# tmuird/VAEUNET

Hardware: AMD Instinct MI355X
Metric: images/sec (whole node) at 3x512x512 bs=8/GPU; Dice parity vs CPU ref (higher is better)
Workload: dtype bf16; 1 GPU; UNet(3,2) train step (fwd+CombinedLoss+bwd+clip+AdamW), random-init weights; image=3x512x512, batch_per_gpu=8, global_batch=8, parallelism=dp1, execution=hipgraph-replay, wgrad_side_stream=False

## Files before the change

include/vaeunet.h:

```cpp
#ifndef VAEUNET_H
#define VAEUNET_H
#include <stdint.h>
#ifdef __cplusplus
extern "C" {
#endif

typedef struct VuGather {
  const void* src[3];
  int64_t stride[3];
  int32_t cend[3];
  int32_t nsrc;
  int32_t C;
  int32_t N, H, W;
  int32_t Hs, Ws;
  int32_t R, S;
  int32_t sy, sx, dy, dx, oy, ox;
} VuGather;

typedef struct VuGemmFwd {
  VuGather a;
  const void* b;
  int64_t ldb;
  int32_t ncol;
  int32_t out_mode;
// ... 170 lines not shown
                     const float* coef2, void* dx1, int64_t dx1s, void* dx2, int64_t dx2s, int dtype,
                     void* stream);
int vu_conv_image_wgrad_bn_ok(int C, int Cp, int64_t das, int64_t ys, int64_t imgs, int N, int H, int W,
                              int dtype);
int vu_conv_image_wgrad_bn_slabs(int N, int H, int W);
int vu_conv_image_wgrad_bn(const void* da, int64_t das, const void* y, int64_t ys, const float* scale,
                           const float* shift, const float* mean, const float* k, int relu,
                           const void* img, int64_t imgs, int N, int H, int W, float* slab, int nslab,
                           void* stream);

int vu_chan_sum(const void* x, int64_t stride, int N, int H, int W, int y0,
                int x0, int Hr, int Wr, int C, float* out, int accumulate,
                float* workspace, int dtype, void* stream);
int64_t vu_reduce_workspace_bytes(int64_t P, int C);
int64_t vu_bn_finalize_workspace_bytes(int tiles, int C);
int vu_zero(void* y, int64_t ys, int64_t P, int C, int dtype, void* stream);
int vu_gpu_delay(int rounds, void* stream);
int vu_zero_insert2(const void* dy, int64_t dys, int N, int h, int w, int C,
                    void* up, int64_t ups, int H, int W, int dtype, void* stream);
int vu_copy(const void* x, int64_t xs, int xdtype, void* y, int64_t ys,
            int ydtype, int64_t P, int C, int accumulate, void* stream);
int vu_input_pack(const float* x, int64_t sn, int64_t sc, int64_t sh,
                  int64_t sw, int N, int C, int H, int W, int Cp, void* y,
                  int dtype, void* stream);

int vu_maxpool2_fwd(const void* x, int64_t xs, int N, int H, int W, int C,
                    void* y, int64_t ys, int dtype, void* stream);
int vu_maxpool2_bwd(const void* x, int64_t xs, const void* dy, int64_t dys,
                    int N, int H, int W, int C, void* dx, int64_t dxs,
                    const void* add, int64_t adds, int dtype, void* stream);
int vu_bn_apply_maxpool2(const void* y, int64_t ys, void* a, int64_t as, void* pool, int64_t ps,
                         int N, int H, int W, int C, const float* scale, const float* shift,
                         int relu, int dtype, void* stream);
int vu_upsample_fwd(const void* x, int64_t xs, int N, int Hi, int Wi, int C,
                    void* y, int64_t ys, int Ho, int Wo, int Hp, int Wp,
                    int py, int px, int dtype, void* stream);
int vu_upsample_bwd(const void* dy, int64_t dys, int N, int Hi, int Wi, int C,
                    void* dx, int64_t dxs, int Ho, int Wo, int Hp, int Wp,
                    int py, int px, int accumulate, int dtype, void* stream);

int64_t vu_attn_tile_rows(void);
int vu_attn_psi_fwd(const void* ug, const void* ux, int64_t P, int F,
                    const float* sg, const float* tg, const float* sx,
                    const float* tx, const float* wpsi, const float* bpsi,
                    float* q, float* psum, float* pm2, int64_t tile_rows,
                    int dtype, void* stream);
int vu_attn_gate_fwd(const float* q, const float* st, const void* x,
                     int64_t xs, int64_t P, int C, float* pmap, void* out,
                     int64_t os, int dtype, void* stream);
int vu_attn_gate_bwd(const void* dout, int64_t dos, const void* x, int64_t xs,
                     const float* pmap, int64_t P, int C, void* dx,
                     int64_t dxs, float* dqpre, int dtype, void* stream);
int64_t vu_attn_psi_bwd_workspace_bytes(int64_t P, int F);
int vu_attn_psi_bwd(const void* ug, const void* ux, int64_t P, int F,
                    const float* sg, const float* tg, const float* sx,
                    const float* tx, const float* wpsi, const float* dq,
                    void* ds, float* dwpsi, float* dbpsi, int accumulate,
                    float* workspace, int dtype, void* stream);
int64_t vu_attn_psi_bwd_blocks(int64_t P);
int vu_attn_psi_bwd_bnb_ok(int F);
int vu_attn_psi_bwd_bnb(const void* ug, const void* ux, int64_t P, int F,
                        const float* sg, const float* tg, const float* sx,
                        const float* tx, const float* wpsi, const float* dq,
                        void* ds, float* dwpsi, float* dbpsi, int accumulate,
                        float* workspace, const float* mean_g, const float* invstd_g,
                        const float* mean_x, const float* invstd_x, float* bnb_g,
// ... 271 lines not shown
```

vaeunet_amd/_lib.py:

```python
import ctypes as C
import os

import torch

_HERE = os.path.dirname(os.path.abspath(__file__))
LIB_PATH = os.path.join(_HERE, "libvaeunet_hip.so")
if os.environ.get("VU_LIB_PATH"):
    LIB_PATH = os.environ["VU_LIB_PATH"]

F32, BF16 = 0, 1

_p = C.c_void_p
_i = C.c_int
_l = C.c_int64
_f = C.c_float


class VuGather(C.Structure):
    _fields_ = [("src", _p * 3), ("stride", _l * 3), ("cend", C.c_int32 * 3),
                ("nsrc", C.c_int32), ("C", C.c_int32),
                ("N", C.c_int32), ("H", C.c_int32), ("W", C.c_int32),
                ("Hs", C.c_int32), ("Ws", C.c_int32), ("R", C.c_int32), ("S", C.c_int32),
                ("sy", C.c_int32), ("sx", C.c_int32), ("dy", C.c_int32), ("dx", C.c_int32),
                ("oy", C.c_int32), ("ox", C.c_int32)]
# ... 84 lines not shown
    "vu_permute4_tile": (_l, []),
    "vu_permute4_batch": (_i, [_p, _i, _l, _p]),
    "vu_permute4_batch2": (_i, [_p, _i, _i, _l, _l, _p]),
    "vu_permute4": (_i, [_p, _l, _l, _l, _l, _l, _i, _i, _i, _i, _i, _p, _i, _p]),
    "vu_bn_finalize": (_i, [_p, _p, _i, _l, _l, _i, _p, _p, _p, _p, _f, _f, _p, _p, _p, _p,
                            _p, _p, _p]),
    "vu_bn_finalize_workspace_bytes": (_l, [_i, _i]),
    "vu_bn_eval_coeffs": (_i, [_p, _p, _p, _p, _f, _i, _p, _p, _p, _p, _p]),
    "vu_bn_apply": (_i, [_p, _l, _p, _l, _l, _i, _p, _p, _i, _i, _p]),
    "vu_bn_fwd_fused_supported": (_i, [_i, _i, _l, _l, _l]),
    "vu_bn_bwd_fused_supported": (_i, [_l, _i, _l, _l, _l]),
    "vu_bn_bwd_fused": (_i, [_p, _l, _p, _l, _l, _i, _p, _p, _p, _p, _p, _i, _i, _p, _p, _i, _p, _l, _p, _i,
                             _p]),
    "vu_bn_fwd_fused": (_i, [_p, _p, _i, _l, _l, _i, _p, _p, _p, _p, _p, _f, _f, _p, _p, _l, _p, _l, _p, _p,
                             _p, _l, _i, _i, _p]),
    "vu_bn_bwd_reduce": (_i, [_p, _l, _p, _l, _l, _i, _p, _p, _p, _p, _p, _i, _i, _p, _p, _i,
                              _p, _p, _i, _p]),
    "vu_bn_bwd_apply": (_i, [_p, _l, _p, _l, _l, _i, _p, _p, _p, _p, _i, _p, _l, _i, _p]),
    "vu_bn_bwd_apply2_ok": (_i, [_i, _l, _l, _l, _l, _l]),
    "vu_bn_bwd_apply2": (_i, [_p, _l, _p, _l, _p, _l, _l, _i, _p, _p, _p, _p, _p, _l, _p, _l, _i, _p]),
    "vu_conv_image_wgrad_bn_ok": (_i, [_i, _i, _l, _l, _l, _i, _i, _i, _i]),
    "vu_conv_image_wgrad_bn_slabs": (_i, [_i, _i, _i]),
    "vu_conv_image_wgrad_bn": (_i, [_p, _l, _p, _l, _p, _p, _p, _p, _i, _p, _l, _i, _i, _i, _p, _i, _p]),
    "vu_reduce_workspace_bytes": (_l, [_l, _i]),
    "vu_chan_sum": (_i, [_p, _l, _i, _i, _i, _i, _i, _i, _i, _i, _p, _i, _p, _i, _p]),
    "vu_copy": (_i, [_p, _l, _i, _p, _l, _i, _l, _i, _i, _p]),
    "vu_zero": (_i, [_p, _l, _l, _i, _i, _p]),
    "vu_gpu_delay": (_i, [_i, _p]),
    "vu_zero_insert2": (_i, [_p, _l, _i, _i, _i, _i, _p, _l, _i, _i, _i, _p]),
    "vu_input_pack": (_i, [_p, _l, _l, _l, _l, _i, _i, _i, _i, _i, _p, _i, _p]),
    "vu_maxpool2_fwd": (_i, [_p, _l, _i, _i, _i, _i, _p, _l, _i, _p]),
    "vu_maxpool2_bwd": (_i, [_p, _l, _p, _l, _i, _i, _i, _i, _p, _l, _p, _l, _i, _p]),
    "vu_bn_apply_maxpool2": (_i, [_p, _l, _p, _l, _p, _l, _i, _i, _i, _i, _p, _p, _i, _i, _p]),
    "vu_upsample_fwd": (_i, [_p, _l, _i, _i, _i, _i, _p, _l, _i, _i, _i, _i, _i, _i, _i, _p]),
    "vu_upsample_bwd": (_i, [_p, _l, _i, _i, _i, _i, _p, _l, _i, _i, _i, _i, _i, _i, _i, _i,
                             _p]),
    "vu_attn_tile_rows": (_l, []),
    "vu_attn_psi_fwd": (_i, [_p, _p, _l, _i, _p, _p, _p, _p, _p, _p, _p, _p, _p, _l, _i, _p]),
    "vu_attn_gate_fwd": (_i, [_p, _p, _p, _l, _l, _i, _p, _p, _l, _i, _p]),
    "vu_attn_gate_bwd": (_i, [_p, _l, _p, _l, _p, _l, _i, _p, _l, _p, _i, _p]),
    "vu_attn_psi_bwd_workspace_bytes": (_l, [_l, _i]),
    "vu_attn_psi_bwd_blocks": (_l, [_l]),
    "vu_attn_psi_bwd_bnb_ok": (_i, [_i]),
    "vu_attn_psi_bwd_bnb": (_i, [_p, _p, _l, _i, _p, _p, _p, _p, _p, _p, _p, _p, _p, _i, _p, _p, _p, _p, _p, _p, _p,
                                 _i, _p]),
    "vu_attn_psi_bwd": (_i, [_p, _p, _l, _i, _p, _p, _p, _p, _p, _p, _p, _p, _p, _i, _p, _i,
                             _p]),
    "vu_attn_tail_bwd_tile": (_l, [_i, _i]),
    "vu_attn_tail_bwd_ok": (_i, [_l, _i, _i, _l, _l, _l, _l, _l, _l, _i]),
    "vu_attn_tail_bwd": (_i, [_p, _p, _p, _l, _i, _i, _p, _p, _p, _p, _p, _p, _p, _p, _p, _p, _l, _p, _l, _p, _l,
                              _p, _p, _l, _l, _i, _p, _l, _p, _p, _i, _p]),
    "vu_pointwise_fwd": (_i, [_p, _l, _l, _i, _i, _p, _p, _p, _l, _i, _p]),
    "vu_pointwise_bwd_workspace_bytes": (_l, [_l, _i, _i]),
    "vu_pointwise_bn_fwd": (_i, [_p, _l, _l, _i, _i, _p, _p, _p, _p, _p, _l, _i, _p]),
    "vu_pointwise_bn_bwd_blocks": (_l, [_l]),
    "vu_pointwise_bn_bwd": (_i, [_p, _l, _p, _l, _p, _l, _l, _i, _i, _p, _p, _l, _p, _p, _i, _p, _p, _i, _p]),
    "vu_pointwise_bwd": (_i, [_p, _l, _p, _l, _l, _i, _i, _p, _p, _l, _p, _p, _i, _p, _i, _p]),
    "vu_loss_workspace_bytes": (_l, []),
    "vu_bce_dice_fwd2": (_i, [_p, _p, _l, _p, _f, _f, _f, _p, _p, _p, _p]),
    "vu_bce_dice_bwd": (_i, [_p, _p, _l, _p, _f, _f, _f, _p, _p, _p]),
    "vu_focal_workspace_bytes": (_l, []),
    "vu_focal_dice_fwd": (_i, [_p, _p, _l, _f, _f, _f, _f, _f, _i, _p, _p, _p, _p, _p]),
    "vu_focal_dice_bwd": (_i, [_p, _p, _l, _f, _f, _f, _f, _f, _i, _p, _p, _p, _p]),
    "vu_kl_free_bits2": (_i, [_p, _p, _i, _i, _f, _p, _p, _p, _p, _p]),
    "vu_sumsq": (_i, [_p, _l, _p, _p, _p]),
    "vu_dice_score": (_i, [_p, _p, _l, _f, _p, _p, _p, _p]),
# ... 95 lines not shown
```

vaeunet_amd/csrc/bn.hip:

```cpp
#include <cstdlib>
#include <type_traits>

#include "host.h"
#include "bn_bwd_elem.h"

namespace {

constexpr int STATS_TPB = 32;
constexpr int STATS_MAXS = 256;

__global__ void bn_stats_stage1(const float* psum, const float* pm2, int tiles, int64_t tile_rows,
                                int64_t rows, int C, int S, double* ws) {
  __shared__ double sh[4][64];
  const int cl = threadIdx.x & 63, tl = threadIdx.x >> 6;
  const int c = blockIdx.x * 64 + cl;
  const bool ok = c < C;
  const int per = (tiles + S - 1) / S;
  const int tb0 = blockIdx.y * per, te0 = min(tiles, tb0 + per);
  constexpr int U = STATS_TPB / 4;
  double N = 0, Mn = 0, Q = 0;
  for (int tb = tb0; tb < te0; tb += STATS_TPB) {
    const int te = min(te0, tb + STATS_TPB);
    const int64_t n_r = min(rows, (int64_t)te * tile_rows) - (int64_t)tb * tile_rows;
    float sv[U], mv[U];
// ... 403 lines not shown
      o2.store(dx2 + p * dx2s + c);
    }
  }
}

template <typename T>
__global__ void bn_bwd_apply_scalar(const T* dy, int64_t dys, const T* x, int64_t xs, int64_t P, int C,
                                    const float* scale, const float* shift, const float* mean,
                                    const float* coef, int relu, T* dx, int64_t dxs) {
  int64_t tot = P * C;
  for (int64_t e = (int64_t)blockIdx.x * blockDim.x + threadIdx.x; e < tot;
       e += (int64_t)gridDim.x * blockDim.x) {
    int64_t p = e / C;
    int c = (int)(e - p * C);
    float xv = ld1<T>(x + p * xs + c), dz = ld1<T>(dy + p * dys + c);
    if (relu && !(fmaf(xv, scale[c], shift[c]) > 0.f)) dz = 0.f;
    st1<T>(dx + p * dxs + c, fmaf(coef[c], dz, coef[C + c] * (xv - mean[c])) + coef[2 * C + c]);
  }
}

template <typename T>
__global__ void bn_apply_scalar(const T* x, int64_t xs, T* y, int64_t ys, int64_t P, int C,
                                const float* scale, const float* shift, int relu) {
  int64_t tot = P * C;
  for (int64_t e = (int64_t)blockIdx.x * blockDim.x + threadIdx.x; e < tot;
       e += (int64_t)gridDim.x * blockDim.x) {
    int64_t p = e / C;
    int c = (int)(e - p * C);
    float z = ld1<T>(x + p * xs + c) * scale[c] + shift[c];
    st1<T>(y + p * ys + c, relu ? fmaxf(z, 0.f) : z);
  }
}

template <typename T>
__global__ void bn_apply_maxpool_kernel(const T* y, int64_t ys, T* a, int64_t as, T* pool, int64_t ps, int N,
                                        int H, int W, int C, const float* scale, const float* shift, int relu) {
  ChanMap cm(C);
  const int c = cm.cv * 8;
  float sc[8], sh[8];
#pragma unroll
  for (int i = 0; i < 8; ++i) { sc[i] = scale[c + i]; sh[i] = shift[c + i]; }
  const int Ho = H >> 1, Wo = W >> 1;
  const int64_t Q = (int64_t)N * Ho * Wo;
  for (int64_t q = (int64_t)blockIdx.x * cm.R + cm.row; q < Q; q += (int64_t)gridDim.x * cm.R) {
    const int j = (int)(q % Wo);
    const int64_t t = q / Wo;
    const int i = (int)(t % Ho), n = (int)(t / Ho);
    const int64_t p00 = ((int64_t)n * H + 2 * i) * W + 2 * j;
    Vec8<T> v[4];
#pragma unroll
    for (int k = 0; k < 4; ++k) v[k].load(y + (p00 + (k >> 1) * W + (k & 1)) * ys + c);
    float best[8];
#pragma unroll
    for (int e = 0; e < 8; ++e) best[e] = -INFINITY;
#pragma unroll
    for (int k = 0; k < 4; ++k) {
#pragma unroll
      for (int e = 0; e < 8; ++e) {
        const float z = v[k].get(e) * sc[e] + sh[e];
        v[k].set(e, relu ? fmaxf(z, 0.f) : z);
        const float f = v[k].get(e);
        if (f > best[e] || isnan(f)) best[e] = f;
      }
      v[k].store(a + (p00 + (k >> 1) * W + (k & 1)) * as + c);
    }
    Vec8<T> o;
#pragma unroll
    for (int e = 0; e < 8; ++e) o.set(e, best[e]);
    o.store(pool + q * ps + c);
  }
}

constexpr int BNF_MAXT = 256;

struct BnFusedArgs {
  const float* psum; const float* pm2; int tiles; int64_t tile_rows; int64_t P; int C;
  const float* gamma; const float* beta; float* rmean; float* rvar; int64_t* nbt; float momentum; float eps;
  float* coef;
  const void* y; int64_t ys;
  const void* res; int64_t rs; const float* rsc; const float* rsh;
  void* out; int64_t os; int relu; int split;
};

template <typename T>
__global__ __launch_bounds__(256) void bn_fwd_fused_kernel(BnFusedArgs a) {
  __shared__ double shd[8][32];
  __shared__ float ssc[32], ssh[32];
  const int cg = blockIdx.x / a.split, sp = blockIdx.x - cg * a.split;
  const int tid = threadIdx.x;
  {
    const int cl = tid & 31, tl = tid >> 5;
    const int c = cg * 32 + cl;
    const float g = a.gamma ? a.gamma[c] : 1.f, b = a.beta ? a.beta[c] : 0.f;
    const bool upd = sp == 0 && a.rmean && a.momentum != 0.f;
    const float rm0 = upd ? a.rmean[c] : 0.f, rv0 = upd ? a.rvar[c] : 0.f;
    const int64_t nb0 = (sp == 0 && a.nbt) ? a.nbt[0] : 0;
    constexpr int U = BNF_MAXT / 8;
    float sv[U], mv[U];
#pragma unroll
    for (int u = 0; u < U; ++u) {
      const int t = min(tl + 8 * u, a.tiles - 1);
      sv[u] = a.psum[(int64_t)t * a.C + c];
// ... 456 lines not shown
                       (const float*)x1, x1s, (const float*)x2, x2s, P, C, mean1, coef1, mean2, coef2, (float*)dx1,
                       dx1s, (float*)dx2, dx2s);
  }
  return (int)hipGetLastError();
}

extern "C" int vu_chan_sum(const void* x, int64_t stride, int N, int H, int W, int y0, int x0, int Hr,
                           int Wr, int C, float* out, int accumulate, float* workspace, int dtype,
                           void* stream) {
  hipStream_t st = (hipStream_t)stream;
  int64_t P = (int64_t)N * Hr * Wr;
  RedArgs r{x, stride, nullptr, 0, P, C, nullptr, nullptr, nullptr, nullptr, 0, workspace, H, W, y0, x0, Hr, Wr};
  int nblk = 0, rc;
  rc = dtype == VU_BF16 ? launch_partial<bf16_t, 0>(r, st, nblk) : launch_partial<float, 0>(r, st, nblk);
  if (rc) return rc;
  hipLaunchKernelGGL(chan_final_sum, dim3((C + 31) / 32), dim3(COLSUM_THREADS), 0, st, workspace, nblk, C, out,
                     accumulate);
  return (int)hipGetLastError();
}

static bool pool_fusable(int H, int W, int C, int64_t s0, int64_t s1, int64_t s2) {
  return H % 2 == 0 && W % 2 == 0 && chanmap_ok(C, s0, s1, s2);
}

extern "C" int vu_bn_apply_maxpool2(const void* y, int64_t ys, void* a, int64_t as, void* pool, int64_t ps, int N,
                                    int H, int W, int C, const float* scale, const float* shift, int relu, int dtype,
                                    void* stream) {
  if (!pool_fusable(H, W, C, ys, as, ps)) return (int)hipErrorInvalidValue;
  const int64_t Q = (int64_t)N * (H / 2) * (W / 2);
  if (Q == 0) return 0;
  const unsigned grid = chan_grid(Q * 4, C, 8192);
  hipStream_t st = (hipStream_t)stream;
  if (dtype == VU_BF16)
    hipLaunchKernelGGL(bn_apply_maxpool_kernel<bf16_t>, dim3(grid), dim3(256), 0, st, (const bf16_t*)y, ys,
                       (bf16_t*)a, as, (bf16_t*)pool, ps, N, H, W, C, scale, shift, relu);
  else
    hipLaunchKernelGGL(bn_apply_maxpool_kernel<float>, dim3(grid), dim3(256), 0, st, (const float*)y, ys,
                       (float*)a, as, (float*)pool, ps, N, H, W, C, scale, shift, relu);
  return (int)hipGetLastError();
}

extern "C" int vu_bn_fwd_fused_supported(int tiles, int C, int64_t ys, int64_t rs, int64_t os) {
  return tiles >= 1 && tiles <= BNF_MAXT && C % 32 == 0 && ys % 8 == 0 && rs % 8 == 0 && os % 8 == 0;
}

extern "C" int vu_bn_fwd_fused(const float* psum, const float* pm2, int tiles, int64_t tile_rows, int64_t P, int C,
                               const float* gamma, const float* beta, float* running_mean, float* running_var,
                               int64_t* num_batches_tracked, float momentum, float eps, float* coef, const void* y,
                               int64_t ys, const void* res, int64_t rs, const float* rscale, const float* rshift,
                               void* out, int64_t os, int relu, int dtype, void* stream) {
  if (!vu_bn_fwd_fused_supported(tiles, C, ys, res ? rs : 0, os) || P < 1) return (int)hipErrorInvalidValue;
  if ((rscale == nullptr) != (rshift == nullptr)) return (int)hipErrorInvalidValue;
  BnFusedArgs a{psum, pm2, tiles, tile_rows, P, C, gamma, beta, running_mean, running_var, num_batches_tracked,
                momentum, eps, coef, y, ys, res, rs, rscale, rshift, out, os, relu, 1};
  const int groups = C / 32;
  int64_t split = (256 + groups - 1) / groups;
  const int64_t maxs = (P + 127) / 128;
  if (split > maxs) split = maxs;
  if (split < 1) split = 1;
  a.split = (int)split;
  hipStream_t st = (hipStream_t)stream;
  if (dtype == VU_BF16)
    hipLaunchKernelGGL(bn_fwd_fused_kernel<bf16_t>, dim3((unsigned)(groups * split)), dim3(256), 0, st, a);
  else
    hipLaunchKernelGGL(bn_fwd_fused_kernel<float>, dim3((unsigned)(groups * split)), dim3(256), 0, st, a);
  return (int)hipGetLastError();
}

extern "C" int vu_bn_bwd_fused_supported(int64_t P, int C, int64_t dys, int64_t xs, int64_t dxs) {
  return C % 32 == 0 && chanmap_ok(C, dys, xs) && dxs % 8 == 0 && P >= 1 &&
         (int)chan_grid16(P, C, RED_MAXBLK) <= BNB_FUSED_MAXBLK;
// ... 29 lines not shown
```

vaeunet_amd/engine.py:

```python
import warnings

import torch

from . import kernels as K
from ._lib import BF16, F32


OVERLAP_WGRAD = False

FUSE_BN_BWD_REDUCE = True


class SideStream:

    _per_device = {}

    def __init__(self, device):
        self.stream = torch.cuda.Stream(device=device)
        self.keep = []
        self.pending = False

    @classmethod
    def get(cls, device):
        key = torch.device(device).index
# ... 292 lines not shown
                                  y, a, relu, M.d, res=res, rcoef=rcoef)
        if coef is not None:
            return coef
    coef = bn_coef(bn, st, C_)
    if res is None:
        K.bn_apply(y, a, coef, relu, M.d)
    else:
        if not relu:
            raise ValueError("bn_fwd_apply: the residual form always applies ReLU (vu_bn_add_relu)")
        N, _, H, W = y.shape
        K.call("vu_bn_add_relu", K.ptr(y), K.pstride(y), K.ptr(coef[0]), K.ptr(coef[1]), K.ptr(res),
               K.pstride(res), K.ptr(rcoef[0]) if rcoef is not None else None,
               K.ptr(rcoef[1]) if rcoef is not None else None, N * H * W, C_, K.ptr(a), K.pstride(a),
               M.d, K.stream())
    return coef


def bn_grad_sinks(bn):
    gw, accw = grad_sink(bn.weight)
    gb, accb = grad_sink(bn.bias)
    if gw is not None and gb is not None and accw != accb:
        raise RuntimeError("inconsistent BatchNorm grad state")
    return gw, gb, accw or accb


def bn_bwd_finish(x, coef, bn, part):
    gw, gb, acc = bn_grad_sinks(bn)
    return K.bn_backward_finish(part, x, coef, bn.weight, gw, gb, acc, train=bn.training)


def bn_bwd(dy, x, coef, bn, relu, M, dx=None, part=None, zrs=None):
    if dx is None:
        dx = torch.empty_like(x)
    if part is not None and part.x is x:
        k = bn_bwd_finish(x, coef, bn, part)
        K.bn_backward_apply(dy, x, coef, k, relu, dx, K.dcode(x.dtype), zrs)
    else:
        gw, gb, acc = bn_grad_sinks(bn)
        K.bn_backward(dy, x, coef, bn.weight, relu, gw, gb, acc, dx, K.dcode(x.dtype),
                      train=bn.training, fused=FUSED_BN_BWD, zrs=zrs)
    return dx


def bn_bwd_pair(dy, a, b, M):
    ka, kb = bn_bwd_finish(*a), bn_bwd_finish(*b)
    (xa, ca, _, _), (xb, cb, _, _) = a, b
    dxa, dxb = torch.empty_like(xa), torch.empty_like(xb)
    if not K.bn_backward_apply2(dy, xa, ca, ka, dxa, xb, cb, kb, dxb, K.dcode(xa.dtype)):
        K.bn_backward_apply(dy, xa, ca, ka, False, dxa, K.dcode(xa.dtype))
        K.bn_backward_apply(dy, xb, cb, kb, False, dxb, K.dcode(xb.dtype))
    return dxa, dxb


FOLD_BN_EVAL = True


def can_fold(M, bn):
    return FOLD_BN_EVAL and M.infer and not bn.training and bn.track_running_stats \
        and bn.running_mean is not None


def fold_bn_eval(M, conv, bn, cin_pad=None, cin_use=None):
    co = conv.out_channels
    coef = bn_coef(bn, None, co)
    img = w3x3_fwd(conv.weight, F32, cin_pad, cin_use)
    w = img * coef[0][:, None]
    if M.d != F32:
# ... 25 lines not shown

def _image_wgrad_kernel_serves(M, srcs, conv, shortcut, da, y):
    if not FUSE_IMAGE_WGRAD_BN or shortcut is not None or M.d != BF16 or K.AUDIT is not None:
        return False
    if len(srcs) != 1 or not conv.weight.requires_grad:
        return False
    return K.image_wgrad_bn_ok(da, y, srcs[0], M.d)


def _image_wgrad_bn_serves(M, srcs, conv, bn, y, da, need_dsrc, da_part, shortcut):
    if need_dsrc or (da_part is not None and da_part.x is not y):
        return False
    N, Cc, H, W = y.shape
    if da_part is None and FUSED_BN_BWD and K.query("vu_bn_bwd_fused_supported", N * H * W, Cc, K.pstride(da),
                                                    K.pstride(y), Cc):
        return False
    return _image_wgrad_kernel_serves(M, srcs, conv, shortcut, da, y)


def _image_wgrad_bn(M, srcs, conv, bn, y, coef, da, cvalid, da_part):
    if da_part is not None:
        k = bn_bwd_finish(y, coef, bn, da_part)
    else:
        gw, gb, acc = bn_grad_sinks(bn)
        k = K.bn_backward_reduce(da, y, coef, bn.weight, True, gw, gb, acc, M.d, train=bn.training)

    def wg():
        g, gacc = grad_sink(conv.weight)
        K.image_wgrad_bn(da, y, coef, k, True, srcs[0], g, conv_layout(g), gacc, cvalid=cvalid)
        M.notify([bn.weight, bn.bias, conv.weight])
    M.side(wg, da, y, k, *srcs)


def conv_bn_relu_bwd(M, srcs, conv, bn, saved, da, need_dsrc, cvalid=None, dsrc=None, dsrc_acc=False,
                     cin_pad=None, da_part=None, feeds=None, shortcut=None):
    y, coef = saved
    if _image_wgrad_bn_serves(M, srcs, conv, bn, y, da, need_dsrc, da_part, shortcut):
        _image_wgrad_bn(M, srcs, conv, bn, y, coef, da, cvalid, da_part)
        return None
    zrs = shortcut.regions(y) if shortcut is not None else None
    dy = bn_bwd(da, y, coef, bn, True, M, part=da_part, zrs=zrs)
    if shortcut is not None:
        shortcut.dy = dy

    def wg():
        if _image_wgrad_kernel_serves(M, srcs, conv, shortcut, dy, dy):
            g, gacc = grad_sink(conv.weight)
            K.image_wgrad_bn(dy, None, None, None, False, srcs[0], g, conv_layout(g), gacc, cvalid=cvalid)
        else:
            wgrad3x3(dy, srcs, conv.weight, M, cvalid, sink=shortcut.sink if shortcut is not None else None)
        M.notify([bn.weight, bn.bias] + ([conv.weight] if shortcut is None else []))
    M.side(wg, dy, *srcs)
    if not need_dsrc:
        return None
    N, _, H, W = y.shape
    cin = shortcut.lead if shortcut is not None else (cin_pad or conv.in_channels)
    if dsrc is None:
        dsrc = M.act(N, cin, H, W)
    bnb = None
    if feeds is not None and FUSE_BN_BWD_REDUCE:
        (fy, fcoef), fbn = feeds
        bnb = (fy, fcoef, True)
    wd = w3x3_dgrad(conv.weight, M.d, rows_use=cin) if shortcut is not None else w3x3_dgrad(conv.weight, M.d, cin)
    part = K.gemm_fwd(K.gather3x3([dy]), wd, cin, dsrc, M.d, accumulate=dsrc_acc, kind="dgrad", bnb=bnb)
    if feeds is not None:
        return dsrc, part
    return dsrc


def double_conv_fwd(M, seq, srcs, cin_pad=None, defer=False):
    conv1, bn1, _, conv2, bn2, _ = seq
    a1, s1 = conv_bn_relu_fwd(M, srcs, conv1, bn1, cin_pad)
    a2, s2 = conv_bn_relu_fwd(M, [a1], conv2, bn2, defer=defer)
    return a2, (srcs, a1, s1, s2)


def double_conv_bwd(M, seq, saved, da2, need_dsrc, cvalid=None, da2_part=None):
    conv1, bn1, _, conv2, bn2, _ = seq
    srcs, a1, s1, s2 = saved
    da1, part = conv_bn_relu_bwd(M, [a1], conv2, bn2, s2, da2, True, feeds=(s1, bn1), da_part=da2_part)
    return conv_bn_relu_bwd(M, srcs, conv1, bn1, s1, da1, need_dsrc, cvalid, da_part=part)


def down_fwd(M, mod, x, pend=None, defer=False):
    seq = mod.maxpool_conv[1].double_conv
    if x is None:
        y, coef = pend
        N, C_, H, W = y.shape
        x = M.act(N, C_, H, W)
        xp = M.act(N, C_, H // 2, W // 2)
        K.bn_apply_maxpool(y, x, xp, coef, True, M.d)
    else:
        xp = K.maxpool_fwd(x, M.d)
    out, sdc = double_conv_fwd(M, seq, [xp], defer=defer)
    return x, out, (x, sdc)


def down_bwd(M, mod, saved, dout, add=None):
    x, sdc = saved
    seq = mod.maxpool_conv[1].double_conv
    dxp = double_conv_bwd(M, seq, sdc, dout, True)
    dx = torch.empty_like(x)
    K.maxpool_bwd(x, dxp, dx, add, M.d)
    return dx


FUSE_ATTN_BN_REDUCE = True
FUSE_ATTN_TAIL = True
ATTN_TAIL_MIN_TILES_PER_CU = 8


def _attn_tail_ok(M, P, F, g, x, dout, dg_out, wdg, wdx, dx):
    if not FUSE_ATTN_TAIL or M.d != BF16 or dg_out is None or g.shape[1] != x.shape[1]:
        return False
    C_ = x.shape[1]
    dst, coff = dg_out
    if not K.query("vu_attn_tail_bwd_ok", P, F, C_, wdg.shape[-1], wdx.shape[-1], K.pstride(dout),
                   K.pstride(dst), coff, K.pstride(dx), M.d):
        return False
    cus = torch.cuda.get_device_properties(x.device).multi_processor_count
    return P // K.query("vu_attn_tail_bwd_tile", F, C_) >= ATTN_TAIL_MIN_TILES_PER_CU * cus


def attention_fwd(M, att, g, x):
    N, _, H, W = x.shape
    P = N * H * W
    wg, bng = att.W_g[0], att.W_g[1]
    wx, bnx = att.W_x[0], att.W_x[1]
    wp, bnp = att.psi[0], att.psi[1]
    F = wg.out_channels
    ug = M.act(N, F, H, W)
    stg = K.gemm_fwd(K.gather1x1([g]), w1x1_fwd(wg.weight, M.d), F, ug, M.d, bias=wg.bias,
                     stats=bng.training)
    ux = M.act(N, F, H, W)
    stx = K.gemm_fwd(K.gather1x1([x]), w1x1_fwd(wx.weight, M.d), F, ux, M.d, bias=wx.bias,
                     stats=bnx.training)
    cg = bn_coef(bng, stg, F)
# ... 225 lines not shown
```

vaeunet_amd/kernels.py:

```python
import ctypes as C

import torch

from . import _lib
from ._lib import ptr, call, query, stream, VuGather, VuGemmFwd, VuGemmWgrad

CL = torch.channels_last


def dcode(dtype):
    if dtype == torch.bfloat16:
        return _lib.BF16
    if dtype == torch.float32:
        return _lib.F32
    raise TypeError(f"unsupported activation dtype {dtype}")


def empty_act(N, Cc, H, W, dtype, device):
    return torch.empty((N, Cc, H, W), dtype=dtype, device=device, memory_format=CL)


def zeros_act(N, Cc, H, W, dtype, device):
    y = torch.empty((N, Cc, H, W), dtype=dtype, device=device, memory_format=CL)
    zero(y)
# ... 547 lines not shown


def input_pack(x, Cp, dtype):
    N, Cc, H, W = x.shape
    if x.dtype != torch.float32:
        x = x.float()
    y = empty_act(N, Cp, H, W, torch.bfloat16 if dtype == _lib.BF16 else torch.float32, x.device)
    s = x.stride()
    call("vu_input_pack", ptr(x), s[0], s[1], s[2], s[3], N, Cc, H, W, Cp, ptr(y), dtype, stream())
    return y


def maxpool_fwd(x, dtype):
    N, Cc, H, W = x.shape
    y = empty_act(N, Cc, H // 2, W // 2, x.dtype, x.device)
    call("vu_maxpool2_fwd", ptr(x), pstride(x), N, H, W, Cc, ptr(y), pstride(y), dtype, stream())
    return y


def maxpool_bwd(x, dy, dx, add, dtype):
    N, Cc, H, W = x.shape
    call("vu_maxpool2_bwd", ptr(x), pstride(x), ptr(dy), pstride(dy), N, H, W, Cc, ptr(dx),
         pstride(dx), ptr(add), pstride(add) if add is not None else 0, dtype, stream())
    return dx


def pool_fusable(y):
    N, Cc, H, W = y.shape
    v = Cc // 8
    return (H % 2 == 0 and W % 2 == 0 and Cc % 8 == 0 and 0 < v <= 256 and v & (v - 1) == 0
            and pstride(y) % 8 == 0)


def bn_apply_maxpool(y, a, pool, coef, relu, dtype):
    N, Cc, H, W = y.shape
    call("vu_bn_apply_maxpool2", ptr(y), pstride(y), ptr(a), pstride(a), ptr(pool), pstride(pool), N, H, W, Cc,
         ptr(coef[0]), ptr(coef[1]), 1 if relu else 0, dtype, stream())
    return a, pool


def upsample_fwd(x, out, Ho, Wo, py, px, dtype):
    N, Cc, Hi, Wi = x.shape
    Hp, Wp = out.shape[2], out.shape[3]
    call("vu_upsample_fwd", ptr(x), pstride(x), N, Hi, Wi, Cc, ptr(out), pstride(out), Ho, Wo,
         Hp, Wp, py, px, dtype, stream())
    return out


def upsample_bwd(dy, dx, Ho, Wo, py, px, accumulate, dtype):
    N, Cc, Hi, Wi = dx.shape
    Hp, Wp = dy.shape[2], dy.shape[3]
    call("vu_upsample_bwd", ptr(dy), pstride(dy), N, Hi, Wi, Cc, ptr(dx), pstride(dx), Ho, Wo,
         Hp, Wp, py, px, 1 if accumulate else 0, dtype, stream())
    return dx


def workspace_f32(nbytes, device):
    return torch.empty(max(1, nbytes // 4 + 1), dtype=torch.float32, device=device)
```

Before: 581.9 images/sec.

## Store maxpool argmax in forward and fuse pool backward into BN backward

The fused BN-apply+maxpool forward kernel now also writes a per-channel uint8 argmax map. Backward returns a lazy PoolGrad instead of materialising the full-resolution maxpool gradient. The BN backward reduce and apply kernels then rebuild the routed gradient on the fly from dxp, argmap and the skip add. This avoids writing and re-reading the full-size dx tensor and skips re-reading the pre-pool activation for the argmax. In exchange it adds an argmap write per down block and falls back to materialising when the fused BN path or other conditions do not apply.

```diff
diff --git a/include/vaeunet.h b/include/vaeunet.h
--- a/include/vaeunet.h
+++ b/include/vaeunet.h
@@ -226,6 +226,20 @@
 int vu_bn_apply_maxpool2(const void* y, int64_t ys, void* a, int64_t as, void* pool, int64_t ps,
                          int N, int H, int W, int C, const float* scale, const float* shift,
                          int relu, int dtype, void* stream);
+int vu_bn_apply_maxpool2_arg(const void* y, int64_t ys, void* a, int64_t as, void* pool, int64_t ps,
+                             void* arg, int64_t args, int N, int H, int W, int C, const float* scale,
+                             const float* shift, int relu, int dtype, void* stream);
+int vu_maxpool2_bwd_arg(const void* dxp, int64_t dps, const void* arg, int64_t args, int N, int H, int W,
+                        int C, void* dx, int64_t dxs, const void* add, int64_t adds, int dtype, void* stream);
+int vu_bn_bwd_reduce_pool_blocks(int N, int H, int W, int C);
+int vu_bn_bwd_reduce_pool(const void* dxp, int64_t dps, const void* arg, int64_t args, const void* add,
+                          int64_t adds, const void* x, int64_t xs, int N, int H, int W, int C,
+                          const float* scale, const float* shift, const float* mean, const float* invstd,
+                          int relu, float* part, int dtype, void* stream);
+int vu_bn_bwd_apply_pool(const void* dxp, int64_t dps, const void* arg, int64_t args, const void* add,
+                         int64_t adds, const void* x, int64_t xs, int N, int H, int W, int C,
+                         const float* scale, const float* shift, const float* mean, const float* coef,
+                         int relu, void* out, int64_t os, int dtype, void* stream);
 int vu_upsample_fwd(const void* x, int64_t xs, int N, int Hi, int Wi, int C,
                     void* y, int64_t ys, int Ho, int Wo, int Hp, int Wp,
                     int py, int px, int dtype, void* stream);
diff --git a/vaeunet_amd/_lib.py b/vaeunet_amd/_lib.py
--- a/vaeunet_amd/_lib.py
+++ b/vaeunet_amd/_lib.py
@@ -140,6 +140,12 @@
     "vu_maxpool2_fwd": (_i, [_p, _l, _i, _i, _i, _i, _p, _l, _i, _p]),
     "vu_maxpool2_bwd": (_i, [_p, _l, _p, _l, _i, _i, _i, _i, _p, _l, _p, _l, _i, _p]),
     "vu_bn_apply_maxpool2": (_i, [_p, _l, _p, _l, _p, _l, _i, _i, _i, _i, _p, _p, _i, _i, _p]),
+    "vu_bn_apply_maxpool2_arg": (_i, [_p, _l, _p, _l, _p, _l, _p, _l, _i, _i, _i, _i, _p, _p, _i, _i, _p]),
+    "vu_maxpool2_bwd_arg": (_i, [_p, _l, _p, _l, _i, _i, _i, _i, _p, _l, _p, _l, _i, _p]),
+    "vu_bn_bwd_reduce_pool_blocks": (_i, [_i, _i, _i, _i]),
+    "vu_bn_bwd_reduce_pool": (_i, [_p, _l, _p, _l, _p, _l, _p, _l, _i, _i, _i, _i, _p, _p, _p, _p, _i, _p, _i, _p]),
+    "vu_bn_bwd_apply_pool": (_i, [_p, _l, _p, _l, _p, _l, _p, _l, _i, _i, _i, _i, _p, _p, _p, _p, _i, _p, _l, _i,
+                                  _p]),
     "vu_upsample_fwd": (_i, [_p, _l, _i, _i, _i, _i, _p, _l, _i, _i, _i, _i, _i, _i, _i, _p]),
     "vu_upsample_bwd": (_i, [_p, _l, _i, _i, _i, _i, _p, _l, _i, _i, _i, _i, _i, _i, _i, _i,
                              _p]),
diff --git a/vaeunet_amd/csrc/bn.hip b/vaeunet_amd/csrc/bn.hip
--- a/vaeunet_amd/csrc/bn.hip
+++ b/vaeunet_amd/csrc/bn.hip
@@ -459,9 +459,10 @@
   }
 }
 
-template <typename T>
+template <typename T, bool ARG>
 __global__ void bn_apply_maxpool_kernel(const T* y, int64_t ys, T* a, int64_t as, T* pool, int64_t ps, int N,
-                                        int H, int W, int C, const float* scale, const float* shift, int relu) {
+                                        int H, int W, int C, const float* scale, const float* shift, int relu,
+                                        uint8_t* arg, int64_t args) {
   ChanMap cm(C);
   const int c = cm.cv * 8;
   float sc[8], sh[8];
@@ -478,8 +479,9 @@
 #pragma unroll
     for (int k = 0; k < 4; ++k) v[k].load(y + (p00 + (k >> 1) * W + (k & 1)) * ys + c);
     float best[8];
-#pragma unroll
-    for (int e = 0; e < 8; ++e) best[e] = -INFINITY;
+    uint32_t am[8];
+#pragma unroll
+    for (int e = 0; e < 8; ++e) { best[e] = -INFINITY; am[e] = 0; }
 #pragma unroll
     for (int k = 0; k < 4; ++k) {
 #pragma unroll
@@ -487,7 +489,7 @@
         const float z = v[k].get(e) * sc[e] + sh[e];
         v[k].set(e, relu ? fmaxf(z, 0.f) : z);
         const float f = v[k].get(e);
-        if (f > best[e] || isnan(f)) best[e] = f;
+        if (f > best[e] || isnan(f)) { best[e] = f; if (ARG) am[e] = k; }
       }
       v[k].store(a + (p00 + (k >> 1) * W + (k & 1)) * as + c);
     }
@@ -495,6 +497,149 @@
 #pragma unroll
     for (int e = 0; e < 8; ++e) o.set(e, best[e]);
     o.store(pool + q * ps + c);
+    if (ARG) {
+      u32x2 w;
+      w[0] = am[0] | (am[1] << 8) | (am[2] << 16) | (am[3] << 24);
+      w[1] = am[4] | (am[5] << 8) | (am[6] << 16) | (am[7] << 24);
+      *reinterpret_cast<u32x2*>(arg + q * args + c) = w;
+    }
+  }
+}
+
+struct PoolArgs {
+  const bf16_t* dxp; int64_t dps;
+  const uint8_t* arg; int64_t args;
+  const bf16_t* add; int64_t adds;
+  int N, H, W, C;
+};
+
+template <bool NT>
+struct PoolWin {
+  Vec8<bf16_t> va[4], vg;
+  u32x2 am;
+  int64_t p00;
+  VU_DEV static int64_t pix(int64_t p00, int W, int ab) { return p00 + (ab >> 1) * W + (ab & 1); }
+  VU_DEV void load(const PoolArgs& r, int64_t q, int c) {
+    const int Ho = r.H >> 1, Wo = r.W >> 1;
+    const int j = (int)(q % Wo);
+    const int64_t t = q / Wo;
+    const int i = (int)(t % Ho), n = (int)(t / Ho);
+    p00 = ((int64_t)n * r.H + 2 * i) * r.W + 2 * j;
+    if (r.add) {
+#pragma unroll
+      for (int ab = 0; ab < 4; ++ab) {
+        const bf16_t* p = r.add + pix(p00, r.W, ab) * r.adds + c;
+        if (NT) va[ab].load_nt(p); else va[ab].load(p);
+      }
+    }
+    const u32x2* pa = reinterpret_cast<const u32x2*>(r.arg + q * r.args + c);
+    if (NT) { vg.load_nt(r.dxp + q * r.dps + c); am = __builtin_nontemporal_load(pa); }
+    else { vg.load(r.dxp + q * r.dps + c); am = *pa; }
+  }
+  VU_DEV float dx(bool has_add, int ab, int k) const {
+    const float o = has_add ? va[ab].get(k) : 0.f;
+    const uint32_t win = (am[k >> 2] >> (8 * (k & 3))) & 0xffu;
+    return win == (uint32_t)ab ? rnd<bf16_t>(o + vg.get(k)) : o;
+  }
+};
+
+template <bool NT>
+__global__ __launch_bounds__(256) void maxpool_bwd_arg_kernel(PoolArgs r, bf16_t* dx, int64_t dxs) {
+  ChanMap cm(r.C);
+  const int c = cm.cv * 8;
+  const bool has_add = r.add != nullptr;
+  const int64_t Q = (int64_t)r.N * (r.H >> 1) * (r.W >> 1);
+  for (int64_t q = (int64_t)blockIdx.x * cm.R + cm.row; q < Q; q += (int64_t)gridDim.x * cm.R) {
+    PoolWin<NT> w;
+    w.load(r, q, c);
+#pragma unroll
+    for (int ab = 0; ab < 4; ++ab) {
+      Vec8<bf16_t> o;
+#pragma unroll
+      for (int k = 0; k < 8; ++k) o.set(k, w.dx(has_add, ab, k));
+      o.store(dx + PoolWin<NT>::pix(w.p00, r.W, ab) * dxs + c);
+    }
+  }
+}
+
+template <bool NT>
+__global__ __launch_bounds__(256) void bn_bwd_reduce_pool_kernel(PoolArgs r, const bf16_t* x, int64_t xs,
+                                                                 const float* scale, const float* shift,
+                                                                 const float* mean, const float* invstd, int relu,
+                                                                 float* part) {
+  __shared__ float sh[2][256 * 8];
+  ChanMap cm(r.C);
+  const int c = cm.cv * 8;
+  const bool has_add = r.add != nullptr;
+  float s0[8], s1[8], sc[8], sf[8], mu[8], is[8];
+#pragma unroll
+  for (int i = 0; i < 8; ++i) {
+    s0[i] = 0.f; s1[i] = 0.f;
+    sc[i] = scale[c + i]; sf[i] = shift[c + i]; mu[i] = mean[c + i]; is[i] = invstd[c + i];
+  }
+  const int64_t Q = (int64_t)r.N * (r.H >> 1) * (r.W >> 1);
+  for (int64_t q = (int64_t)blockIdx.x * cm.R + cm.row; q < Q; q += (int64_t)gridDim.x * cm.R) {
+    PoolWin<NT> w;
+    w.load(r, q, c);
+    Vec8<bf16_t> vx[4];
+#pragma unroll
+    for (int ab = 0; ab < 4; ++ab) {
+      const bf16_t* p = x + PoolWin<NT>::pix(w.p00, r.W, ab) * xs + c;
+      if (NT) vx[ab].load_nt(p); else vx[ab].load(p);
+    }
+#pragma unroll
+    for (int ab = 0; ab < 4; ++ab) {
+#pragma unroll
+      for (int i = 0; i < 8; ++i) {
+        const float xv = vx[ab].get(i);
+        float dz = w.dx(has_add, ab, i);
+        if (relu && !(fmaf(xv, sc[i], sf[i]) > 0.f)) dz = 0.f;
+        s0[i] += dz;
+        s1[i] += dz * ((xv - mu[i]) * is[i]);
+      }
+    }
+  }
+#pragma unroll
+  for (int i = 0; i < 8; ++i) { sh[0][cm.row * r.C + c + i] = s0[i]; sh[1][cm.row * r.C + c + i] = s1[i]; }
+  __syncthreads();
+  for (int cc = threadIdx.x; cc < r.C; cc += 256) {
+    part[((int64_t)blockIdx.x * 2 + 0) * r.C + cc] = lds_sum(&sh[0][cc], cm.R, r.C);
+    part[((int64_t)blockIdx.x * 2 + 1) * r.C + cc] = lds_sum(&sh[1][cc], cm.R, r.C);
+  }
+}
+
+template <bool NT>
+__global__ __launch_bounds__(256) void bn_bwd_apply_pool_kernel(PoolArgs r, const bf16_t* x, int64_t xs,
+                                                                const float* scale, const float* shift,
+                                                                const float* mean, const float* coef, int relu,
+                                                                bf16_t* out, int64_t os) {
+  ChanMap cm(r.C);
+  const int c = cm.cv * 8;
+  const bool has_add = r.add != nullptr;
+  float sc[8], sf[8], mu[8], k1[8], k2[8], k3[8];
+#pragma unroll
+  for (int i = 0; i < 8; ++i) {
+    sc[i] = scale[c + i]; sf[i] = shift[c + i]; mu[i] = mean[c + i];
+    k1[i] = coef[c + i]; k2[i] = coef[r.C + c + i]; k3[i] = coef[2 * r.C + c + i];
+  }
+  const int64_t Q = (int64_t)r.N * (r.H >> 1) * (r.W >> 1);
+  for (int64_t q = (int64_t)blockIdx.x * cm.R + cm.row; q < Q; q += (int64_t)gridDim.x * cm.R) {
+    PoolWin<NT> w;
+    w.load(r, q, c);
+    Vec8<bf16_t> vx[4];
+#pragma unroll
+    for (int ab = 0; ab < 4; ++ab) {
+      const bf16_t* p = x + PoolWin<NT>::pix(w.p00, r.W, ab) * xs + c;
+      if (NT) vx[ab].load_nt(p); else vx[ab].load(p);
+    }
+#pragma unroll
+    for (int ab = 0; ab < 4; ++ab) {
+      Vec8<bf16_t> o;
+#pragma unroll
+      for (int i = 0; i < 8; ++i)
+        o.set(i, bn_bwd_elem(vx[ab].get(i), w.dx(has_add, ab, i), relu, sc[i], sf[i], mu[i], k1[i], k2[i], k3[i]));
+      o.store(out + PoolWin<NT>::pix(w.p00, r.W, ab) * os + c);
+    }
   }
 }
 
@@ -1017,11 +1162,94 @@
   const unsigned grid = chan_grid(Q * 4, C, 8192);
   hipStream_t st = (hipStream_t)stream;
   if (dtype == VU_BF16)
-    hipLaunchKernelGGL(bn_apply_maxpool_kernel<bf16_t>, dim3(grid), dim3(256), 0, st, (const bf16_t*)y, ys,
-                       (bf16_t*)a, as, (bf16_t*)pool, ps, N, H, W, C, scale, shift, relu);
+    hipLaunchKernelGGL((bn_apply_maxpool_kernel<bf16_t, false>), dim3(grid), dim3(256), 0, st, (const bf16_t*)y, ys,
+                       (bf16_t*)a, as, (bf16_t*)pool, ps, N, H, W, C, scale, shift, relu, (uint8_t*)nullptr,
+                       (int64_t)0);
   else
-    hipLaunchKernelGGL(bn_apply_maxpool_kernel<float>, dim3(grid), dim3(256), 0, st, (const float*)y, ys,
-                       (float*)a, as, (float*)pool, ps, N, H, W, C, scale, shift, relu);
+    hipLaunchKernelGGL((bn_apply_maxpool_kernel<float, false>), dim3(grid), dim3(256), 0, st, (const float*)y, ys,
+                       (float*)a, as, (float*)pool, ps, N, H, W, C, scale, shift, relu, (uint8_t*)nullptr,
+                       (int64_t)0);
+  return (int)hipGetLastError();
+}
+
+static bool pool_arg_ok(int H, int W, int C, int64_t args, int64_t s0, int64_t s1, int64_t s2, int dtype) {
+  return dtype == VU_BF16 && args % 8 == 0 && args >= C && pool_fusable(H, W, C, s0, s1, s2);
+}
+
+extern "C" int vu_bn_apply_maxpool2_arg(const void* y, int64_t ys, void* a, int64_t as, void* pool, int64_t ps,
+                                        void* arg, int64_t args, int N, int H, int W, int C, const float* scale,
+                                        const float* shift, int relu, int dtype, void* stream) {
+  if (!arg || !pool_arg_ok(H, W, C, args, ys, as, ps, dtype)) return (int)hipErrorInvalidValue;
+  const int64_t Q = (int64_t)N * (H / 2) * (W / 2);
+  if (Q == 0) return 0;
+  hipLaunchKernelGGL((bn_apply_maxpool_kernel<bf16_t, true>), dim3(chan_grid(Q * 4, C, 8192)), dim3(256), 0,
+                     (hipStream_t)stream, (const bf16_t*)y, ys, (bf16_t*)a, as, (bf16_t*)pool, ps, N, H, W, C, scale,
+                     shift, relu, (uint8_t*)arg, args);
+  return (int)hipGetLastError();
+}
+
+extern "C" int vu_maxpool2_bwd_arg(const void* dxp, int64_t dps, const void* arg, int64_t args, int N, int H, int W,
+                                   int C, void* dx, int64_t dxs, const void* add, int64_t adds, int dtype,
+                                   void* stream) {
+  if (!arg || !pool_arg_ok(H, W, C, args, dps, dxs, add ? adds : 8, dtype)) return (int)hipErrorInvalidValue;
+  const int64_t Q = (int64_t)N * (H / 2) * (W / 2);
+  if (Q == 0) return 0;
+  const PoolArgs r{(const bf16_t*)dxp, dps, (const uint8_t*)arg, args, (const bf16_t*)add, adds, N, H, W, C};
+  const unsigned grid = chan_grid(Q * 4, C, 8192);
+  if (bn_nt(Q * 4, C, 2))
+    hipLaunchKernelGGL(maxpool_bwd_arg_kernel<true>, dim3(grid), dim3(256), 0, (hipStream_t)stream, r, (bf16_t*)dx, dxs);
+  else
+    hipLaunchKernelGGL(maxpool_bwd_arg_kernel<false>, dim3(grid), dim3(256), 0, (hipStream_t)stream, r, (bf16_t*)dx, dxs);
+  return (int)hipGetLastError();
+}
+
+extern "C" int vu_bn_bwd_reduce_pool_blocks(int N, int H, int W, int C) {
+  if (C < 8 || C % 8 || !pow2(C / 8) || C / 8 > 256) return 0;
+  const int64_t Q = (int64_t)N * (H / 2) * (W / 2);
+  if (Q <= 0) return 0;
+  static int resident = 0;
+  if (resident == 0) {
+    int b = 0;
+    if (hipOccupancyMaxActiveBlocksPerMultiprocessor(&b, bn_bwd_reduce_pool_kernel<true>, 256, 0) != hipSuccess || b < 1)
+      b = 2;
+    resident = b * cu_count();
+  }
+  const int g = (int)chan_grid(Q * 4, C, RED_MAXBLK);
+  return g < resident ? g : resident;
+}
+
+extern "C" int vu_bn_bwd_reduce_pool(const void* dxp, int64_t dps, const void* arg, int64_t args, const void* add,
+                                     int64_t adds, const void* x, int64_t xs, int N, int H, int W, int C,
+                                     const float* scale, const float* shift, const float* mean, const float* invstd,
+                                     int relu, float* part, int dtype, void* stream) {
+  if (!arg || !pool_arg_ok(H, W, C, args, dps, xs, add ? adds : 8, dtype)) return (int)hipErrorInvalidValue;
+  const int nblk = vu_bn_bwd_reduce_pool_blocks(N, H, W, C);
+  if (nblk < 1) return (int)hipErrorInvalidValue;
+  const PoolArgs r{(const bf16_t*)dxp, dps, (const uint8_t*)arg, args, (const bf16_t*)add, adds, N, H, W, C};
+  if (bn_nt((int64_t)N * H * W, C, 2))
+    hipLaunchKernelGGL(bn_bwd_reduce_pool_kernel<true>, dim3(nblk), dim3(256), 0, (hipStream_t)stream, r,
+                       (const bf16_t*)x, xs, scale, shift, mean, invstd, relu, part);
+  else
+    hipLaunchKernelGGL(bn_bwd_reduce_pool_kernel<false>, dim3(nblk), dim3(256), 0, (hipStream_t)stream, r,
+                       (const bf16_t*)x, xs, scale, shift, mean, invstd, relu, part);
+  return (int)hipGetLastError();
+}
+
+extern "C" int vu_bn_bwd_apply_pool(const void* dxp, int64_t dps, const void* arg, int64_t args, const void* add,
+                                    int64_t adds, const void* x, int64_t xs, int N, int H, int W, int C,
+                                    const float* scale, const float* shift, const float* mean, const float* coef,
+                                    int relu, void* out, int64_t os, int dtype, void* stream) {
+  if (!arg || os % 8 || !pool_arg_ok(H, W, C, args, dps, xs, add ? adds : 8, dtype)) return (int)hipErrorInvalidValue;
+  const int64_t Q = (int64_t)N * (H / 2) * (W / 2);
+  if (Q == 0) return 0;
+  const PoolArgs r{(const bf16_t*)dxp, dps, (const uint8_t*)arg, args, (const bf16_t*)add, adds, N, H, W, C};
+  const unsigned grid = chan_grid(Q * 4, C, 8192);
+  if (bn_nt(Q * 4, C, 2))
+    hipLaunchKernelGGL(bn_bwd_apply_pool_kernel<true>, dim3(grid), dim3(256), 0, (hipStream_t)stream, r,
+                       (const bf16_t*)x, xs, scale, shift, mean, coef, relu, (bf16_t*)out, os);
+  else
+    hipLaunchKernelGGL(bn_bwd_apply_pool_kernel<false>, dim3(grid), dim3(256), 0, (hipStream_t)stream, r,
+                       (const bf16_t*)x, xs, scale, shift, mean, coef, relu, (bf16_t*)out, os);
   return (int)hipGetLastError();
 }
 
diff --git a/vaeunet_amd/engine.py b/vaeunet_amd/engine.py
--- a/vaeunet_amd/engine.py
+++ b/vaeunet_amd/engine.py
@@ -348,7 +348,11 @@
 def bn_bwd(dy, x, coef, bn, relu, M, dx=None, part=None, zrs=None):
     if dx is None:
         dx = torch.empty_like(x)
-    if part is not None and part.x is x:
+    if isinstance(dy, PoolGrad):
+        part = K.bn_backward_reduce_pool(dy.dxp, dy.arg, dy.add, x, coef, relu, M.d)
+        k = bn_bwd_finish(x, coef, bn, part)
+        K.bn_backward_apply_pool(dy.dxp, dy.arg, dy.add, x, coef, k, relu, dx, M.d)
+    elif part is not None and part.x is x:
         k = bn_bwd_finish(x, coef, bn, part)
         K.bn_backward_apply(dy, x, coef, k, relu, dx, K.dcode(x.dtype), zrs)
     else:
@@ -440,9 +444,19 @@
     M.side(wg, da, y, k, *srcs)
 
 
+def _pool_bn_bwd_serves(M, y, da, need_dsrc, da_part, shortcut):
+    if not need_dsrc or da_part is not None or shortcut is not None or M.d != BF16 or K.AUDIT is not None:
+        return False
+    N, Cc, H, W = y.shape
+    return not (FUSED_BN_BWD and K.query("vu_bn_bwd_fused_supported", N * H * W, Cc, K.pstride(da.x),
+                                         K.pstride(y), Cc))
+
+
 def conv_bn_relu_bwd(M, srcs, conv, bn, saved, da, need_dsrc, cvalid=None, dsrc=None, dsrc_acc=False,
                      cin_pad=None, da_part=None, feeds=None, shortcut=None):
     y, coef = saved
+    if isinstance(da, PoolGrad) and not _pool_bn_bwd_serves(M, y, da, need_dsrc, da_part, shortcut):
+        da = da.materialise(M)
     if _image_wgrad_bn_serves(M, srcs, conv, bn, y, da, need_dsrc, da_part, shortcut):
         _image_wgrad_bn(M, srcs, conv, bn, y, coef, da, cvalid, da_part)
         return None
@@ -490,27 +504,43 @@
     return conv_bn_relu_bwd(M, srcs, conv1, bn1, s1, da1, need_dsrc, cvalid, da_part=part)
 
 
+FUSE_POOL_BN_BWD = 2
+
+
+class PoolGrad:
+
+    def __init__(self, dxp, arg, add, x):
+        self.dxp, self.arg, self.add, self.x = dxp, arg, add, x
+
+    def materialise(self, M):
+        return K.maxpool_bwd_arg(self.dxp, self.arg, torch.empty_like(self.x), self.add, M.d)
+
+
 def down_fwd(M, mod, x, pend=None, defer=False):
     seq = mod.maxpool_conv[1].double_conv
+    arg = None
     if x is None:
         y, coef = pend
         N, C_, H, W = y.shape
         x = M.act(N, C_, H, W)
         xp = M.act(N, C_, H // 2, W // 2)
-        K.bn_apply_maxpool(y, x, xp, coef, True, M.d)
+        if FUSE_POOL_BN_BWD and M.d == BF16 and not M.infer:
+            arg = K.pool_argmap(y)
+        K.bn_apply_maxpool(y, x, xp, coef, True, M.d, arg=arg)
     else:
         xp = K.maxpool_fwd(x, M.d)
     out, sdc = double_conv_fwd(M, seq, [xp], defer=defer)
-    return x, out, (x, sdc)
+    return x, out, (x, sdc, arg)
 
 
 def down_bwd(M, mod, saved, dout, add=None):
-    x, sdc = saved
+    x, sdc, arg = saved
     seq = mod.maxpool_conv[1].double_conv
     dxp = double_conv_bwd(M, seq, sdc, dout, True)
-    dx = torch.empty_like(x)
-    K.maxpool_bwd(x, dxp, dx, add, M.d)
-    return dx
+    if arg is None or not FUSE_POOL_BN_BWD:
+        return K.maxpool_bwd(x, dxp, torch.empty_like(x), add, M.d)
+    g = PoolGrad(dxp, arg, add, x)
+    return g if FUSE_POOL_BN_BWD == 2 else g.materialise(M)
 
 
 FUSE_ATTN_BN_REDUCE = True
diff --git a/vaeunet_amd/kernels.py b/vaeunet_amd/kernels.py
--- a/vaeunet_amd/kernels.py
+++ b/vaeunet_amd/kernels.py
@@ -603,11 +603,47 @@
             and pstride(y) % 8 == 0)
 
 
-def bn_apply_maxpool(y, a, pool, coef, relu, dtype):
+def bn_apply_maxpool(y, a, pool, coef, relu, dtype, arg=None):
     N, Cc, H, W = y.shape
+    if arg is not None:
+        call("vu_bn_apply_maxpool2_arg", ptr(y), pstride(y), ptr(a), pstride(a), ptr(pool), pstride(pool),
+             ptr(arg), arg.shape[-1], N, H, W, Cc, ptr(coef[0]), ptr(coef[1]), 1 if relu else 0, dtype, stream())
+        return a, pool
     call("vu_bn_apply_maxpool2", ptr(y), pstride(y), ptr(a), pstride(a), ptr(pool), pstride(pool), N, H, W, Cc,
          ptr(coef[0]), ptr(coef[1]), 1 if relu else 0, dtype, stream())
     return a, pool
+
+
+def pool_argmap(y):
+    N, Cc, H, W = y.shape
+    return torch.empty((N, H // 2, W // 2, Cc), dtype=torch.uint8, device=y.device)
+
+
+def _pool_seam(dxp, arg, add):
+    return (ptr(dxp), pstride(dxp), ptr(arg), arg.shape[-1], ptr(add), pstride(add) if add is not None else 0)
+
+
+def maxpool_bwd_arg(dxp, arg, dx, add, dtype):
+    N, Cc, H, W = dx.shape
+    call("vu_maxpool2_bwd_arg", ptr(dxp), pstride(dxp), ptr(arg), arg.shape[-1], N, H, W, Cc, ptr(dx), pstride(dx),
+         ptr(add), pstride(add) if add is not None else 0, dtype, stream())
+    return dx
+
+
+def bn_backward_reduce_pool(dxp, arg, add, x, coef, relu, dtype):
+    N, Cc, H, W = x.shape
+    nblk = query("vu_bn_bwd_reduce_pool_blocks", N, H, W, Cc)
+    part = torch.empty(max(1, nblk) * 2 * Cc, dtype=torch.float32, device=x.device)
+    call("vu_bn_bwd_reduce_pool", *_pool_seam(dxp, arg, add), ptr(x), pstride(x), N, H, W, Cc, ptr(coef[0]),
+         ptr(coef[1]), ptr(coef[2]), ptr(coef[3]), 1 if relu else 0, ptr(part), dtype, stream())
+    return BnbPart(part, nblk, x)
+
+
+def bn_backward_apply_pool(dxp, arg, add, x, coef, k, relu, out, dtype):
+    N, Cc, H, W = x.shape
+    call("vu_bn_bwd_apply_pool", *_pool_seam(dxp, arg, add), ptr(x), pstride(x), N, H, W, Cc, ptr(coef[0]),
+         ptr(coef[1]), ptr(coef[2]), ptr(k), 1 if relu else 0, ptr(out), pstride(out), dtype, stream())
+    return out
 
 
 def upsample_fwd(x, out, Ho, Wo, py, px, dtype):
```

New measurement: 587.7 images/sec (median of 6 runs). Within noise of the previous version (+1.0%).
